# 666DZY666/micronet

Measured on AMD Instinct MI355X. Metric: QAT images/sec (nin_gc CIFAR-10, W-ternary/A-binary), higher is better.
Workload: dtype f32

## Files before the change

### include/micronet_hip.h

```cpp
#ifndef MICRONET_HIP_H
#define MICRONET_HIP_H

#include <stddef.h>
#include <stdint.h>

#ifdef __cplusplus
extern "C" {
#endif

#define MN_OK 0
#define MN_EINVAL (-22)
#define MN_ENOTSUP (-95)
#define MN_EHIP (-5)
#define MN_ENOSPC (-28)

typedef void* mn_stream_t;

int mn_version(void);
const char* mn_last_error(void);
const char* mn_last_kernel(void);
void mn_profile_next(void* start_event, void* stop_event);
typedef struct mn_prof_entry {
    char name[96];
    int64_t launches;
// ... 268 lines not shown
                                const float* sums, int training, const float* w, float* dx, void* ws, int64_t ws_bytes, mn_stream_t stream);
int mn_conv2d_bwd_weight_bnh_pool(const mn_conv_geom* g, const float* dpool, const uint8_t* h, const int8_t* own, const float* chan, const float* sums,
                                  int training, const int8_t* x, float* dw, float* dbias, void* ws, int64_t ws_bytes, mn_stream_t stream);
int mn_conv2d_bwd_bnh_supported(const mn_conv_geom* g, const mn_wq* wq, int pooled);
int64_t mn_conv2d_bwd_bnh_ws_bytes(const mn_conv_geom* g);
int mn_conv2d_bwd_bnh(const mn_conv_geom* g, const mn_wq* wq, const float* da, const uint8_t* h, const int8_t* own, const float* chan, const float* sums,
                      int training, const float* w, const int8_t* x, float* dx, float* dw, float* dbias, void* ws, int64_t ws_bytes, mn_stream_t stream);
int mn_conv2d_bwd_bnh_up_splits(const mn_conv_geom* g, const mn_wq* wq, int pooled, int64_t up_k);
int mn_conv2d_bwd_bnh_up(const mn_conv_geom* g, const mn_wq* wq, const float* da, const uint8_t* h, const int8_t* own, const float* chan, const float* sums,
                         int training, const float* w, const int8_t* x, float* dx, float* dw, float* dbias, void* ws, int64_t ws_bytes,
                         const uint8_t* up_h, const float* up_chan, double* up_part, mn_stream_t stream);
int mn_conv2d_bwd_bnh_up9_splits(const mn_conv_geom* g, const mn_wq* wq, int64_t up_k);
int mn_conv2d_bwd_bnh_up9(const mn_conv_geom* g, const mn_wq* wq, const float* da, const uint8_t* h, const float* chan, const float* sums, int training,
                          const float* w, const int8_t* x, float* dx, float* dw, float* dbias, void* ws, int64_t ws_bytes, const uint8_t* up_h, const float* up_chan,
                          double* up_part, mn_stream_t stream);
int mn_conv2d_bwd_codes(const mn_conv_geom* g, const mn_wq* wq, const float* gy, const float* w, const void* x_codes, int x_bits, float* dx, float* dw, float* dbias,
                        void* ws, int64_t ws_bytes, mn_stream_t stream);
int mn_conv2d_bwd_qa(const mn_conv_geom* g, const mn_wq* wq, const float* dq, const void* stash, int stash_bits, const float* chan, const float* sums, int out_bits,
                     int quant, int training, const float* w, const uint8_t* x_codes, int x_bits, float* dx, float* dw, float* dbias, void* ws, int64_t ws_bytes,
                     mn_stream_t stream);
int mn_conv2d_bwd_codes_up(const mn_conv_geom* g, const mn_wq* wq, const float* gy, const float* w, const void* x_codes, int x_bits, float* dx, float* dw, float* dbias,
                           void* ws, int64_t ws_bytes, const void* up_stash, const float* up_chan, int up_quant, double* up_part, mn_stream_t stream);
int mn_conv2d_bwd_qa_up(const mn_conv_geom* g, const mn_wq* wq, const float* dq, const void* stash, const float* chan, const float* sums, int out_bits, int quant,
                        int training, const float* w, const uint8_t* x_codes, int x_bits, float* dx, float* dw, float* dbias, void* ws, int64_t ws_bytes,
                        const void* up_stash, const float* up_chan, int up_quant, double* up_part, mn_stream_t stream);
int mn_qconv_bnsign_bwd_pooled(const mn_conv_geom* g, const mn_wq* wq, const int8_t* x, const float* w, const float* bias, const float* gamma,
                               const float* beta, const float* save, const float* dpool, const int8_t* a_own, int training, float* dy,
                               float* dgamma, float* dbeta, void* ws, int64_t ws_bytes, mn_stream_t stream);

#define MN_QA_NCH 9
// ... 118 lines not shown
```

### micronet_amd/_lib.py

```python
import ctypes as C
import os

HERE = os.path.dirname(os.path.abspath(__file__))
LIB_PATH = os.environ.get("MN_LIB_PATH") or os.path.join(HERE, "lib", "libmicronet_hip.so")

MN_ACTQ_NONE, MN_ACTQ_DOREFA, MN_ACTQ_IAO, MN_ACTQ_SIGN8, MN_ACTQ_CODE8 = 0, 1, 2, 3, 4
MN_ALGO_AUTO, MN_ALGO_DIRECT, MN_ALGO_MFMA, MN_ALGO_QGEMM = 0, 1, 2, 3
MN_WQ_REAL, MN_WQ_TERNARY, MN_WQ_DOREFA, MN_WQ_IAO = 0, 1, 2, 3
MN_ACTQ_X_IS_CODE = 1
MN_ACTQ_CODES_GIVEN = 2
MN_ENOTSUP = -95


class ConvGeom(C.Structure):
    _fields_ = [(n, C.c_int32) for n in ("N", "C", "H", "W", "O", "KH", "KW", "stride_h", "stride_w", "pad_h", "pad_w",
                                         "dil_h", "dil_w", "groups", "in_shuffle")]


class ActQ(C.Structure):
    _fields_ = [("mode", C.c_int32), ("bits", C.c_int32), ("q_type", C.c_int32), ("flags", C.c_int32),
                ("qp", C.c_void_p), ("codes", C.c_void_p), ("stats", C.c_void_p), ("dx_add", C.c_void_p), ("ste_mask", C.c_void_p), ("acc_mm", C.c_void_p)]


class WQ(C.Structure):
# ... 84 lines not shown
    "mn_qconv_bnsign_fwd_stash_pool_supported": (_I, [_G, _W]),
    "mn_qconv_bnsign_fwd_stash_pool": (_I, [_G, _W, _P, _P, _P, _P, _P, C.c_float, C.c_float, _I, _P, _P, _P, _P, _P, _P, _P, _P, _P, _L, _P]),
    "mn_bnh_bwd_sums": (_I, [_P, _P, _P, _P, _L, _L, _L, _L, _P, _P, _P, _P, _P]),
    "mn_bnh_bwd_apply": (_I, [_P, _P, _P, _P, _P, _L, _L, _L, _L, _I, _P, _P]),
    "mn_conv2d_bnh_supported": (_I, [_G, _W]),
    "mn_conv2d_bwd_data_bnh": (_I, [_G, _W, _P, _P, _P, _P, _I, _P, _P, _P, _L, _P]),
    "mn_conv2d_bwd_weight_bnh": (_I, [_G, _P, _P, _P, _P, _I, _P, _P, _P, _P, _L, _P]),
    "mn_conv2d_bwd_bnh_supported": (_I, [_G, _W, _I]),
    "mn_conv2d_bwd_bnh_ws_bytes": (_L, [_G]),
    "mn_conv2d_bwd_bnh": (_I, [_G, _W, _P, _P, _P, _P, _P, _I, _P, _P, _P, _P, _P, _P, _L, _P]),
    "mn_conv2d_bwd_bnh_up_splits": (_I, [_G, _W, _I, _L]),
    "mn_conv2d_bwd_bnh_up": (_I, [_G, _W, _P, _P, _P, _P, _P, _I, _P, _P, _P, _P, _P, _P, _L, _P, _P, _P, _P]),
    "mn_bnh_bwd_sums_final": (_I, [_P, _I, _L, _L, _L, _L, _P, _P, _P, _P]),
    "mn_conv2d_bwd_bnh_up9_splits": (_I, [_G, _W, _L]),
    "mn_conv2d_bwd_bnh_up9": (_I, [_G, _W, _P, _P, _P, _P, _I, _P, _P, _P, _P, _P, _P, _L, _P, _P, _P, _P]),
    "mn_conv2d_bwd_codes": (_I, [_G, _W, _P, _P, _P, _I, _P, _P, _P, _P, _L, _P]),
    "mn_conv2d_bwd_qa": (_I, [_G, _W, _P, _P, _I, _P, _P, _I, _I, _I, _P, _P, _I, _P, _P, _P, _P, _L, _P]),
    "mn_conv2d_bwd_codes_up": (_I, [_G, _W, _P, _P, _P, _I, _P, _P, _P, _P, _L, _P, _P, _I, _P, _P]),
    "mn_conv2d_bwd_qa_up": (_I, [_G, _W, _P, _P, _P, _P, _I, _I, _I, _P, _P, _I, _P, _P, _P, _P, _L, _P, _P, _I, _P, _P]),
    "mn_qa_bwd_sums_final": (_I, [_P, _I, _L, _P, _P, _P, _P]),
    "mn_conv2d_bnh_pool_supported": (_I, [_G, _W]),
    "mn_conv2d_bwd_data_bnh_pool": (_I, [_G, _W, _P, _P, _P, _P, _P, _I, _P, _P, _P, _L, _P]),
    "mn_conv2d_bwd_weight_bnh_pool": (_I, [_G, _P, _P, _P, _P, _P, _I, _P, _P, _P, _P, _L, _P]),
    "mn_qconv_bnsign_bwd": (_I, [_G, _W, _P, _P, _P, _P, _P, _P, _P, _I, _P, _P, _P, _P, _L, _P]),
    "mn_qconv_bnsign_bwd_pooled": (_I, [_G, _W, _P, _P, _P, _P, _P, _P, _P, _P, _I, _P, _P, _P, _P, _L, _P]),
    "mn_signconv1x1_small_supported": (_I, [_L, _L, _L]),
    "mn_signconv1x1_small_fwd": (_I, [_P, _P, _P, _P, _L, _L, _L, _L, _P]),
    "mn_codeconv1x1_small_fwd": (_I, [_P, _I, _P, _P, _P, _L, _L, _L, _L, _P]),
    "mn_conv1x1_small_bwd_data": (_I, [_P, _P, _P, _L, _L, _L, _L, _P]),
    "mn_iao_fq_act_fwd": (_I, [_P, _P, _L, _P, _I, _I, _I, C.c_float, _P]),
# ... 152 lines not shown
```

### micronet_amd/csrc/conv_kernels.hip

```cpp
#include "common.h"
#include "qgemm.h"

#define EPI_PLAIN 0
#define EPI_BIAS 1
#define EPI_STE 2

struct TileGeom {
    int TP, NI, TR, tpi;
    int PR, PW, HALO, CS;
    int num_ptiles;
    FastDiv fd_wo, fd_tr, fd_pwq, fd_pr, fd_ni, fd_tpi, fd_ppi;
    int tpq_shift;
};
struct ConvView {
    const float* in;
    int N, Cin_total, Hin, Win, U, Hv, Wv, Kc, G;
    int Cout_total, Ho, Wo, Mg;
    int KH, KW, Sh, Sw, Dh, Dw, ph, pw;
    int vec_in;
};
static inline int roundup(int a, int b) { return (a + b - 1) / b * b; }

static int make_tile_geom(const ConvView& v, int TP, int cs_mod32, TileGeom* t) {
    if (v.Wo < 4 || TP % v.Wo != 0 || v.pw > 8 || v.pw < 0 || v.ph < 0) return 0;
// ... 797 lines not shown
    return pwb_bwd_bnh_up(g, wq, da, h, own, chan, sums, training, w, x, dx, dw, dbias, ws, ws_bytes, up_h, up_chan, up_part, (hipStream_t)stream);
}
extern "C" int mn_conv2d_bwd_bnh_up9_splits(const mn_conv_geom* g, const mn_wq* wq, int64_t up_k) {
    if (check_geom(g, "mn_conv2d_bwd_bnh_up9_splits") != MN_OK) return 0;
    if (up_k < 1 || up_k > 254 || !pwb_supported(g, wq, 0)) return 0;
    return pwb_up9_splits(g);
}
extern "C" int mn_conv2d_bwd_bnh_up9(const mn_conv_geom* g, const mn_wq* wq, const float* da, const uint8_t* h, const float* chan, const float* sums, int training,
                                     const float* w, const int8_t* x, float* dx, float* dw, float* dbias, void* ws, int64_t ws_bytes, const uint8_t* up_h,
                                     const float* up_chan, double* up_part, mn_stream_t stream) {
    int rc = check_geom(g, "mn_conv2d_bwd_bnh_up9");
    if (rc) return rc;
    if (!wq || !da || !h || !chan || !sums || !w || !x || !dx || !dw || !up_h || !up_chan || !up_part) MN_FAIL(MN_EINVAL, "mn_conv2d_bwd_bnh_up9: null tensor");
    return pwb_bwd_bnh_up9(g, wq, da, h, chan, sums, training, w, x, dx, dw, dbias, ws, ws_bytes, up_h, up_chan, up_part, (hipStream_t)stream);
}
extern "C" int mn_conv2d_bwd_codes(const mn_conv_geom* g, const mn_wq* wq, const float* gy, const float* w, const void* x_codes, int x_bits, float* dx, float* dw,
                                   float* dbias, void* ws, int64_t ws_bytes, mn_stream_t stream) {
    int rc = check_geom(g, "mn_conv2d_bwd_codes");
    if (rc) return rc;
    if (!wq || !gy || !w || !x_codes || !dx || !dw || x_bits < 0 || x_bits > 8) MN_FAIL(MN_EINVAL, "mn_conv2d_bwd_codes: null tensor / bad bit width");
    return pwb_bwd_plain(g, wq, gy, w, x_codes, x_bits, dx, dw, dbias, ws, ws_bytes, (hipStream_t)stream);
}
extern "C" int mn_conv2d_bwd_qa(const mn_conv_geom* g, const mn_wq* wq, const float* dq, const void* stash, int stash_bits, const float* chan, const float* sums,
                                int out_bits, int quant, int training, const float* w, const uint8_t* x_codes, int x_bits, float* dx, float* dw, float* dbias, void* ws,
                                int64_t ws_bytes, mn_stream_t stream) {
    int rc = check_geom(g, "mn_conv2d_bwd_qa");
    if (rc) return rc;
    if (!wq || !dq || !stash || !chan || !sums || !w || !x_codes || !dx || !dw) MN_FAIL(MN_EINVAL, "mn_conv2d_bwd_qa: null tensor");
    return pwb_bwd_qa(g, wq, dq, stash, stash_bits, chan, sums, out_bits, quant, training, w, x_codes, x_bits, dx, dw, dbias, ws, ws_bytes, (hipStream_t)stream);
}
// ... 126 lines not shown
```

### micronet_amd/csrc/qgemm.h

```cpp
#pragma once
#include "common.h"

int qg_supported(const mn_conv_geom* g, const mn_actq* aq, const mn_wq* wq, int which);
int64_t qg_ws_bytes(const mn_conv_geom* g, int which);
int qg_fwd(const mn_conv_geom* g, const mn_actq* aq, const mn_wq* wq, const float* x, const float* w, const float* bias, float* y,
           void* ws, int64_t ws_bytes, hipStream_t s);
int qg_bwd_data(const mn_conv_geom* g, const mn_actq* aq, const mn_wq* wq, const float* gy, const float* w, const float* x, float* dx,
                void* ws, int64_t ws_bytes, hipStream_t s);
int qg_fwd_act_mm_count(const mn_conv_geom* g);
int qg_fwd_act(const mn_conv_geom* g, const mn_actq* aq, const mn_wq* wq, const float* x, const float* w, const float* bias, float* y, int relu, float* mm,
               void* ws, int64_t ws_bytes, hipStream_t s);
int c1_supported(const mn_conv_geom* g, int which);
int64_t c1_ws_bytes(const mn_conv_geom* g, int which);
int c1_fwd(const mn_conv_geom* g, const float* x, const float* w, const float* bias, float* y, void* ws, int64_t ws_bytes, hipStream_t s);
int c1_fwd_mm_count(const mn_conv_geom* g);
int c1_fwd_act(const mn_conv_geom* g, const float* x, const float* w, const float* bias, float* y, int relu, float* mm, void* ws, int64_t ws_bytes, hipStream_t s);
int c1_bwd_weight_bn(const mn_conv_geom* g, const float* gy, const float* da, const float* yb, const float* save, const float* gamma, const float* beta,
                     const float* sums, int training, const float* x, float* dw, float* dbias, void* ws, int64_t ws_bytes, hipStream_t s);
int c1_bwd_weight(const mn_conv_geom* g, const float* gy, const float* x, float* dw, float* dbias, void* ws, int64_t ws_bytes, hipStream_t s);
int c1_bwd_weight_qa(const mn_conv_geom* g, const float* dq, const float* yb, const float* chan, int quant, int a_bits, const float* sums, int training,
                     const float* x, float* dw, float* dbias, void* ws, int64_t ws_bytes, hipStream_t s);
int qd_iao_dx_add_supported(const mn_conv_geom* g, const mn_actq* aq, const mn_wq* wq);
int64_t qd_iao_ws_bytes(const mn_conv_geom* g, int which);
int qd_iao_bwd_data(const mn_conv_geom* g, const mn_actq* aq, const mn_wq* wq, const float* gy, const float* w, const float* x, float* dx, void* ws, int64_t ws_bytes,
// ... 29 lines not shown
int pwb_up_splits(const mn_conv_geom* g);
int pwb_bwd_bnh_up(const mn_conv_geom* g, const mn_wq* wq, const float* da, const uint8_t* h, const int8_t* own, const float* chan, const float* sums, int training,
                   const float* w, const int8_t* x, float* dx, float* dw, float* dbias, void* ws, int64_t ws_bytes, const uint8_t* up_h, const float* up_chan,
                   double* up_part, hipStream_t s);
int pwb_up9_splits(const mn_conv_geom* g);
int pwb_bwd_bnh_up9(const mn_conv_geom* g, const mn_wq* wq, const float* da, const uint8_t* h, const float* chan, const float* sums, int training, const float* w,
                    const int8_t* x, float* dx, float* dw, float* dbias, void* ws, int64_t ws_bytes, const uint8_t* up_h, const float* up_chan, double* up_part,
                    hipStream_t s);
int pwb_bwd_plain_up(const mn_conv_geom* g, const mn_wq* wq, const float* gy, const float* w, const void* x, int x_bits, float* dx, float* dw, float* dbias, void* ws,
                     int64_t ws_bytes, const void* up_stash, const float* up_chan, int up_quant, double* up_part, hipStream_t s);
int pwb_bwd_qa_up(const mn_conv_geom* g, const mn_wq* wq, const float* dq, const void* stash, const float* chan, const float* sums, int out_bits, int quant, int training,
                  const float* w, const uint8_t* x, int x_bits, float* dx, float* dw, float* dbias, void* ws, int64_t ws_bytes, const void* up_stash, const float* up_chan,
                  int up_quant, double* up_part, hipStream_t s);
int pwb_bwd_bnh(const mn_conv_geom* g, const mn_wq* wq, const float* da, const uint8_t* h, const int8_t* own, const float* chan, const float* sums, int training,
                const float* w, const int8_t* x, float* dx, float* dw, float* dbias, void* ws, int64_t ws_bytes, hipStream_t s);
int pwb_bwd_plain(const mn_conv_geom* g, const mn_wq* wq, const float* gy, const float* w, const void* x, int x_bits, float* dx, float* dw, float* dbias, void* ws,
                  int64_t ws_bytes, hipStream_t s);
int pwb_bwd_qa(const mn_conv_geom* g, const mn_wq* wq, const float* dq, const void* stash, int stash_bits, const float* chan, const float* sums, int out_bits, int quant,
               int training, const float* w, const uint8_t* x, int x_bits, float* dx, float* dw, float* dbias, void* ws, int64_t ws_bytes, hipStream_t s);
```

### micronet_amd/csrc/qgemm_k3s.hip

```cpp
#include "qgemm_dev.h"

#include <stdlib.h>

#define K3_RSA 160
#define K3_NXL 6

struct K3wParams {
    const float* gy;
    const char* x;
    float* part;
    float* dbpart;
    int N, C, H, W, O, Cg, Mg, G, nmb, ncb, Z, Mgw, Cgw, want_db;
    int R, spi, nsteps, st_per_z, DPC, W4, CS, XB;
    FastDiv fd_spi, fd_dpc, fd_w4;
    ChanMap in_map;
};

template <int XENC>
__global__ __launch_bounds__(256, 2) void k_k3s_wgrad(const K3wParams p) {
    HIP_DYNAMIC_SHARED(float, smem)
    const int tid = threadIdx.x, lane = tid & 63, wave = tid >> 6, j = lane & 15, kg = lane >> 4;
    unsigned char* gsm = reinterpret_cast<unsigned char*>(smem) + wave * (32 * K3_RSA + p.XB);
    unsigned char* xsm = gsm + 32 * K3_RSA;
    uint32_t b = blockIdx.x;
// ... 768 lines not shown
    p.wn = (float)((1ll << wq->bits) - 1);
    mn_set_last_kernel(wide ? "k_k3s_fwd<2>" : "k_k3s_fwd<1>");
    { const double nx = (double)g->N * g->C * g->H * g->W, ny = (double)g->N * g->O * g->H * g->W; mn_prof_bytes(nx + (wide ? 4.0 : 2.0) * ny); }
    mn_prof_begin(s);
    if (wide) {
        raise_lds_limit((const void*)k_k3s_fwd<2>, pl.lds);
        hipLaunchKernelGGL(k_k3s_fwd<2>, dim3(pl.grid), dim3(256), pl.lds, s, p);
    } else {
        raise_lds_limit((const void*)k_k3s_fwd<1>, pl.lds);
        hipLaunchKernelGGL(k_k3s_fwd<1>, dim3(pl.grid), dim3(256), pl.lds, s, p);
    }
    mn_prof_end(s);
    MN_CHECK_LAUNCH("mn_qconv_bnq_fwd_stash(3x3)");
    return MN_OK;
}
```

### micronet_amd/ops.py

```python
import ctypes as C
import threading
import weakref

import torch
from torch.autograd import Function

from . import _lib
from ._lib import ActQ, ConvGeom, MicronetHipError, WQ
from .sign_tensor import LazyBNAct, LazyBNGrad, LazyConvOut, LazyPoolGrad, LazyQConvOut, LazyReluConvOut, LazyReluGrad, QActTensor, QGrad, SignTensor

ACTQ_NONE, ACTQ_DOREFA, ACTQ_IAO, ACTQ_SIGN8, ACTQ_CODE8 = _lib.MN_ACTQ_NONE, _lib.MN_ACTQ_DOREFA, _lib.MN_ACTQ_IAO, _lib.MN_ACTQ_SIGN8, _lib.MN_ACTQ_CODE8
WQ_REAL, WQ_TERNARY, WQ_DOREFA, WQ_IAO = _lib.MN_WQ_REAL, _lib.MN_WQ_TERNARY, _lib.MN_WQ_DOREFA, _lib.MN_WQ_IAO

PROFILER = None


class _Span:
    __slots__ = ("tok",)

    def __init__(self, tok):
        self.tok = tok

    def __enter__(self):
        return self
# ... 1765 lines not shown


def _out_hw(g):
    return ((g.H + 2 * g.pad_h - g.dil_h * (g.KH - 1) - 1) // g.stride_h + 1,
            (g.W + 2 * g.pad_w - g.dil_w * (g.KW - 1) - 1) // g.stride_w + 1)


def _ws(g, which, device):
    nb = int(_lib_().mn_conv2d_ws_bytes(C.byref(g), which, _lib.MN_ALGO_AUTO))
    if nb < 0:
        raise MicronetHipError("invalid convolution geometry")
    return torch.empty(max(nb // 4, 4), dtype=torch.float32, device=device), nb


FUSE_PW_BWD = _os0.environ.get("MN_PWB", "1") != "0"


def _wq_desc(wdesc):
    if wdesc is None:
        return None
    mode, bits, q_type, per_channel, scale = wdesc
    return WQ(mode, bits, q_type, per_channel, scale.data_ptr() if scale is not None else None)


def _ref(d):
    return None if d is None else C.byref(d)


class UpSums:
    __slots__ = ("h", "chan", "k", "ready", "kind")
# ... 78 lines not shown
            elif _lib_().mn_conv2d_bwd_data_add_supported(C.byref(g), C.byref(aq), C.byref(wd)):
                ctx.res_tok = x._mn_res_token = ResidualToken()
        ctx.save_for_backward(x, wq, qp, wscale)
        ctx.cfg = (g, aq_mode, aq_bits, aq_qtype, bias is not None, wdesc[:4] if wdesc is not None else None, aq_flags)
        return y

    @staticmethod
    def backward(ctx, gy):
        x, wq, qp, wscale = ctx.saved_tensors
        g, aq_mode, aq_bits, aq_qtype, has_bias, wd4, aq_flags = ctx.cfg
        if isinstance(gy, LazyBNGrad) and gy._mn_value is None and gy._mn_recipe.get("kind") == "first_done":
            r = gy._mn_recipe
            if aq_mode == ACTQ_NONE and not ctx.needs_input_grad[0] and r["x"].data_ptr() == x.data_ptr() and r["w"].data_ptr() == wq.data_ptr() and \
                    tuple(r["dw"].shape) == tuple(wq.shape) and (not has_bias or r["db"] is not None):
                return None, r["dw"], (r["db"] if has_bias else None), None, None, None, None, None, None, None, None, None, None, None, None
        if isinstance(gy, LazyBNGrad) and gy._mn_value is None and gy._mn_recipe.get("kind") in ("bnh", "bnh_pool") and aq_mode == ACTQ_SIGN8 and wd4 is not None:
            r = gy._mn_recipe
            pool = r.get("kind") == "bnh_pool"
            wd = _wq_desc(wd4 + (wscale,))
            if getattr(ctx, "packed", None) is not None and ctx.packed[1] is not None:
                wd.packed_bwd = ctx.packed[1].data_ptr()
            dx = dw = db = None
            want_w = ctx.needs_input_grad[1] or (has_bias and ctx.needs_input_grad[2])
            if ctx.needs_input_grad[0] and want_w and FUSE_PW_BWD and _lib_().mn_conv2d_bwd_bnh_supported(C.byref(g), _ref(wd), 1 if pool else 0) and \
                    r["da"].data_ptr() % 16 == 0 and x.data_ptr() % 16 == 0:
                with torch.cuda.device_of(x):
                    dx = torch.empty(x.shape, dtype=torch.float32, device=x.device)
                    dw = torch.empty_like(wq)
                    db = torch.empty(g.O, dtype=torch.float32, device=x.device) if has_bias else None
                    nb = int(_lib_().mn_conv2d_bwd_bnh_ws_bytes(C.byref(g)))
                    ws = torch.empty(max(nb // 4, 4), dtype=torch.float32, device=x.device)
# ... 166 lines not shown
            wd.packed_fwd = pk[0].data_ptr()
        with torch.cuda.device_of(codes):
            nb = int(_lib_().mn_qconv_bnsign_stash_ws_bytes(C.byref(g)))
            ws = torch.empty(nb // 4 + 4, dtype=torch.float32, device=codes.device)
            ap = None
            if pool_next and training and POOL_IN_SIGN_PASS and a.data_ptr() % 16 == 0 and h.data_ptr() % 16 == 0 and \
                    _lib_().mn_qconv_bnsign_fwd_stash_pool_supported(C.byref(g), _ref(wd)):
                ap = torch.empty((y.shape[0], y.shape[1], y.shape[2] // 2, y.shape[3] // 2), dtype=torch.int8, device=codes.device)
                _call("mn_qconv_bnsign_fwd_stash_pool", C.byref(g), _ref(wd), _p(codes), _p(wq), _p(bias), _p(gamma), _p(beta), float(eps), float(momentum),
                      int(training), _p(running_mean), _p(running_var), _p(nbt), _p(save), _p(a), _p(ap), _p(h), _p(chan), _p(ws), nb, _s())
            else:
                _call("mn_qconv_bnsign_fwd_stash", C.byref(g), _ref(wd), _p(codes), _p(wq), _p(bias), _p(gamma), _p(beta), float(eps), float(momentum),
                      int(training), _p(running_mean), _p(running_var), _p(nbt), _p(save), _p(a), _p(h), _p(chan), _p(ws), nb, _s())
        ctx.save_for_backward(h, chan, gamma, beta)
        ctx.training = int(training)
        ctx.fold_ok = FOLD_BN_INTO_CONV_BWD and bool(_lib_().mn_conv2d_bnh_supported(C.byref(g), _ref(wd)))
        ctx.fold_pool_ok = ctx.fold_ok and bool(_lib_().mn_conv2d_bnh_pool_supported(C.byref(g), _ref(wd)))
        out = SignTensor(a)
        if ap is not None:
            out._mn_pooled = ap
        ctx.up_rec = None
        if chan.shape[0] in (8, 17) and UP_SUMS_FOLD:
            ctx.up_rec = out._mn_up = UpSums(h, chan, wq.shape[1] * wq.shape[2] * wq.shape[3], kind=1 if chan.shape[0] == 8 else 3)
        return out

    @staticmethod
    def backward(ctx, da):
        h, chan, gamma, beta = ctx.saved_tensors
        training = ctx.training
        pooled = isinstance(da, LazyPoolGrad) and da._mn_value is None
        if pooled:
            grad, own = da._mn_pg, da._mn_codes
# ... 15 lines not shown
                _call("mn_bnh_bwd_sums", _p(grad), _p(h), _p(own), _p(chan), N, Cc, H, W, _p(dgamma), _p(dbeta), _p(sums), _p(ws), _s())
            if pooled and getattr(ctx, "fold_pool_ok", False) and LAZY_BN_GRAD:
                def expand_p(r):
                    dy_ = torch.empty(r["h"].shape, dtype=torch.float32, device=r["h"].device)
                    with torch.cuda.device_of(dy_):
                        _call("mn_bnh_bwd_apply", _p(r["da"]), _p(r["h"]), _p(r["own"]), _p(r["chan"]), _p(r["sums"]), N, Cc, H, W, r["training"], _p(dy_), _s())
                    return dy_
                recipe = dict(kind="bnh_pool", da=grad, own=own, h=h, chan=chan, sums=sums, training=training)
                return LazyBNGrad(h.shape, h.device, recipe, expand_p), dgamma, dbeta, None, None, None, None, None, None, None
            if not pooled and ctx.fold_ok and LAZY_BN_GRAD:
                def expand(r):
                    dy_ = torch.empty(r["h"].shape, dtype=torch.float32, device=r["h"].device)
                    with torch.cuda.device_of(dy_):
                        _call("mn_bnh_bwd_apply", _p(r["da"]), _p(r["h"]), None, _p(r["chan"]), _p(r["sums"]), N, Cc, H, W, r["training"], _p(dy_), _s())
                    return dy_
                recipe = dict(kind="bnh", da=grad, h=h, chan=chan, sums=sums, training=training)
                return LazyBNGrad(h.shape, h.device, recipe, expand), dgamma, dbeta, None, None, None, None, None, None, None
            dy = torch.empty(h.shape, dtype=torch.float32, device=h.device)
            _call("mn_bnh_bwd_apply", _p(grad), _p(h), _p(own), _p(chan), _p(sums), N, Cc, H, W, training, _p(dy), _s())
        return dy, dgamma, dbeta, None, None, None, None, None, None, None


def qconv_bnq_supported(x, wq, stride, padding, dilation, groups, w_bits, in_shuffle):
    if not isinstance(x, QActTensor) or x.dim() != 4 or not (2 <= w_bits <= 8):
        return False
    one = lambda v: v in (1, (1, 1), [1, 1])
    if not one(dilation):
        return False
    g = _geom(x.shape, wq.shape, stride, padding, dilation, groups, in_shuffle or 0)
    wd = WQ(WQ_DOREFA, w_bits, 0, 0, None)
    return bool(_lib_().mn_qconv_bnq_supported(C.byref(g), C.byref(wd), x.bits))
# ... 835 lines not shown
```

Before: 145,000.

## Fuse BN-backward apply into 3x3 ternary conv backward data and weight kernel

Adds a fused kernel for 3x3 stride-1 grouped ternary convolutions. It rebuilds the BN/hardtanh input gradient from the stashed codes and per-channel stats inside the conv backward, then computes dx through bf16 MFMA with a three-way bf16 split, while other waves accumulate weight-gradient partials. The Python side marks eligible BN layers so the lazy BN gradient is never materialized for them. This removes a full-size float dy write and read plus separate dgrad/wgrad launches, at the cost of a large specialized kernel with narrow geometry limits and a high LDS footprint.

```diff
diff --git a/include/micronet_hip.h b/include/micronet_hip.h
--- a/include/micronet_hip.h
+++ b/include/micronet_hip.h
@@ -306,6 +306,10 @@
 int mn_conv2d_bwd_bnh_up9(const mn_conv_geom* g, const mn_wq* wq, const float* da, const uint8_t* h, const float* chan, const float* sums, int training,
                           const float* w, const int8_t* x, float* dx, float* dw, float* dbias, void* ws, int64_t ws_bytes, const uint8_t* up_h, const float* up_chan,
                           double* up_part, mn_stream_t stream);
+int mn_conv2d_bwd_bnh_k3_supported(const mn_conv_geom* g, const mn_wq* wq);
+int64_t mn_conv2d_bwd_bnh_k3_ws_bytes(const mn_conv_geom* g);
+int mn_conv2d_bwd_bnh_k3(const mn_conv_geom* g, const mn_wq* wq, const float* da, const uint8_t* h, const float* chan, const float* sums, int training,
+                         const float* w, const int8_t* x, float* dx, float* dw, float* dbias, void* ws, int64_t ws_bytes, mn_stream_t stream);
 int mn_conv2d_bwd_codes(const mn_conv_geom* g, const mn_wq* wq, const float* gy, const float* w, const void* x_codes, int x_bits, float* dx, float* dw, float* dbias,
                         void* ws, int64_t ws_bytes, mn_stream_t stream);
 int mn_conv2d_bwd_qa(const mn_conv_geom* g, const mn_wq* wq, const float* dq, const void* stash, int stash_bits, const float* chan, const float* sums, int out_bits,
diff --git a/micronet_amd/_lib.py b/micronet_amd/_lib.py
--- a/micronet_amd/_lib.py
+++ b/micronet_amd/_lib.py
@@ -122,6 +122,9 @@
     "mn_bnh_bwd_sums_final": (_I, [_P, _I, _L, _L, _L, _L, _P, _P, _P, _P]),
     "mn_conv2d_bwd_bnh_up9_splits": (_I, [_G, _W, _L]),
     "mn_conv2d_bwd_bnh_up9": (_I, [_G, _W, _P, _P, _P, _P, _I, _P, _P, _P, _P, _P, _P, _L, _P, _P, _P, _P]),
+    "mn_conv2d_bwd_bnh_k3_supported": (_I, [_G, _W]),
+    "mn_conv2d_bwd_bnh_k3_ws_bytes": (_L, [_G]),
+    "mn_conv2d_bwd_bnh_k3": (_I, [_G, _W, _P, _P, _P, _P, _I, _P, _P, _P, _P, _P, _P, _L, _P]),
     "mn_conv2d_bwd_codes": (_I, [_G, _W, _P, _P, _P, _I, _P, _P, _P, _P, _L, _P]),
     "mn_conv2d_bwd_qa": (_I, [_G, _W, _P, _P, _I, _P, _P, _I, _I, _I, _P, _P, _I, _P, _P, _P, _P, _L, _P]),
     "mn_conv2d_bwd_codes_up": (_I, [_G, _W, _P, _P, _P, _I, _P, _P, _P, _P, _L, _P, _P, _I, _P, _P]),
diff --git a/micronet_amd/csrc/conv_kernels.hip b/micronet_amd/csrc/conv_kernels.hip
--- a/micronet_amd/csrc/conv_kernels.hip
+++ b/micronet_amd/csrc/conv_kernels.hip
@@ -835,6 +835,21 @@
     if (!wq || !da || !h || !chan || !sums || !w || !x || !dx || !dw || !up_h || !up_chan || !up_part) MN_FAIL(MN_EINVAL, "mn_conv2d_bwd_bnh_up9: null tensor");
     return pwb_bwd_bnh_up9(g, wq, da, h, chan, sums, training, w, x, dx, dw, dbias, ws, ws_bytes, up_h, up_chan, up_part, (hipStream_t)stream);
 }
+extern "C" int mn_conv2d_bwd_bnh_k3_supported(const mn_conv_geom* g, const mn_wq* wq) {
+    if (check_geom(g, "mn_conv2d_bwd_bnh_k3_supported") != MN_OK) return 0;
+    return k3b_supported(g, wq);
+}
+extern "C" int64_t mn_conv2d_bwd_bnh_k3_ws_bytes(const mn_conv_geom* g) {
+    if (check_geom(g, "mn_conv2d_bwd_bnh_k3_ws_bytes") != MN_OK) return -1;
+    return k3b_ws_bytes(g);
+}
+extern "C" int mn_conv2d_bwd_bnh_k3(const mn_conv_geom* g, const mn_wq* wq, const float* da, const uint8_t* h, const float* chan, const float* sums, int training,
+                                    const float* w, const int8_t* x, float* dx, float* dw, float* dbias, void* ws, int64_t ws_bytes, mn_stream_t stream) {
+    int rc = check_geom(g, "mn_conv2d_bwd_bnh_k3");
+    if (rc) return rc;
+    if (!wq || !da || !h || !chan || !sums || !w || !x || !dx || !dw) MN_FAIL(MN_EINVAL, "mn_conv2d_bwd_bnh_k3: null tensor");
+    return k3b_bwd_bnh(g, wq, da, h, chan, sums, training, w, x, dx, dw, dbias, ws, ws_bytes, (hipStream_t)stream);
+}
 extern "C" int mn_conv2d_bwd_codes(const mn_conv_geom* g, const mn_wq* wq, const float* gy, const float* w, const void* x_codes, int x_bits, float* dx, float* dw,
                                    float* dbias, void* ws, int64_t ws_bytes, mn_stream_t stream) {
     int rc = check_geom(g, "mn_conv2d_bwd_codes");
diff --git a/micronet_amd/csrc/qgemm.h b/micronet_amd/csrc/qgemm.h
--- a/micronet_amd/csrc/qgemm.h
+++ b/micronet_amd/csrc/qgemm.h
@@ -67,6 +67,10 @@
                   int up_quant, double* up_part, hipStream_t s);
 int pwb_bwd_bnh(const mn_conv_geom* g, const mn_wq* wq, const float* da, const uint8_t* h, const int8_t* own, const float* chan, const float* sums, int training,
                 const float* w, const int8_t* x, float* dx, float* dw, float* dbias, void* ws, int64_t ws_bytes, hipStream_t s);
+int k3b_supported(const mn_conv_geom* g, const mn_wq* wq);
+int64_t k3b_ws_bytes(const mn_conv_geom* g);
+int k3b_bwd_bnh(const mn_conv_geom* g, const mn_wq* wq, const float* da, const uint8_t* h, const float* chan, const float* sums, int training, const float* w,
+                const int8_t* x, float* dx, float* dw, float* dbias, void* ws, int64_t ws_bytes, hipStream_t s);
 int pwb_bwd_plain(const mn_conv_geom* g, const mn_wq* wq, const float* gy, const float* w, const void* x, int x_bits, float* dx, float* dw, float* dbias, void* ws,
                   int64_t ws_bytes, hipStream_t s);
 int pwb_bwd_qa(const mn_conv_geom* g, const mn_wq* wq, const float* dq, const void* stash, int stash_bits, const float* chan, const float* sums, int out_bits, int quant,
diff --git a/micronet_amd/csrc/qgemm_k3s.hip b/micronet_amd/csrc/qgemm_k3s.hip
--- a/micronet_amd/csrc/qgemm_k3s.hip
+++ b/micronet_amd/csrc/qgemm_k3s.hip
@@ -806,3 +806,423 @@
     MN_CHECK_LAUNCH("mn_qconv_bnq_fwd_stash(3x3)");
     return MN_OK;
 }
+
+#define K3B_FR 20
+
+struct K3bParams {
+    const float* da;
+    const unsigned char* h;
+    const float* chan;
+    const float* sums;
+    const char* x;
+    const float* w;
+    float* dx;
+    float* part;
+    float* dbpart;
+    int N, C, H, W, O, Cg, Mg, G, Z, training, want_db;
+    float n_f;
+    int NI, SP, HW, IS, TS, WP, RS32;
+    int nsteps, st_per_z, spi;
+    FastDiv fd_hw4, fd_w4, fd_w;
+    ChanMap in_map;
+};
+
+__global__ __launch_bounds__(512, 1) void k_k3b(const K3bParams p) {
+    HIP_DYNAMIC_SHARED(float, smem)
+    unsigned char* lds = reinterpret_cast<unsigned char*>(smem);
+    unsigned char* dyr = lds + 3 * p.TS;
+    float* ftab = reinterpret_cast<float*>(dyr + 32 * p.RS32);
+    const int tid = threadIdx.x, lane = tid & 63, wave = mn_uniform(tid >> 6), j = lane & 15, kg = lane >> 4;
+    const int role = wave >> 2, rw = wave & 3;
+    const uint32_t b = blockIdx.x;
+    const int z = (int)(b % (uint32_t)p.Z);
+    const int g = (int)(b / (uint32_t)p.Z);
+    const int wrow = p.Cg * 9;
+
+    float* wl = reinterpret_cast<float*>(lds);
+    for (int i = tid; i < p.Mg * wrow; i += 512) wl[i] = p.w[(int64_t)g * p.Mg * wrow + i];
+    __syncthreads();
+    float my_alpha = 0.f;
+    u32x4 wa[9];
+    if (role == 0) {
+        {
+            const int m = tid >> 3, part = tid & 7;
+            float a = 0.f;
+            if (m < p.Mg) for (int k = part; k < wrow; k += 8) a = fmaxf(a, fabsf(wl[m * wrow + k]));
+            a = fmaxf(a, __shfl_xor(a, 4, 64)); a = fmaxf(a, __shfl_xor(a, 2, 64)); a = fmaxf(a, __shfl_xor(a, 1, 64));
+            my_alpha = a;
+        }
+        const int c = j;
+#pragma unroll
+        for (int t = 0; t < 9; ++t) {
+            uint32_t h16[8];
+#pragma unroll
+            for (int e = 0; e < 8; ++e) {
+                const int m = 2 * kg + (e >> 2) + 8 * (e & 3);
+                float v = 0.f;
+                if (m < p.Mg && c < p.Cg) v = wl[m * wrow + c * 9 + t];
+                h16[e] = v > 0.f ? 0x3F80u : (v < 0.f ? 0xBF80u : 0u);
+            }
+            wa[t] = u32x4{h16[0] | (h16[1] << 16), h16[2] | (h16[3] << 16), h16[4] | (h16[5] << 16), h16[6] | (h16[7] << 16)};
+        }
+    }
+    __syncthreads();
+    for (int i = tid; i < (3 * p.TS) / 16; i += 512) *reinterpret_cast<u32x4*>(lds + 16 * i) = u32x4{0u, 0u, 0u, 0u};
+    if (role == 0 && (tid & 7) == 0) {
+        const int m = tid >> 3, co = g * p.Mg + (m < p.Mg ? m : p.Mg - 1), O = p.O;
+        float* fr = ftab + m * K3B_FR;
+        const StashNnz zn = stash_nnz_load(p.chan, O, co);
+        const bool ok = m < p.Mg;
+        fr[0] = ok ? p.chan[O + co] : 0.f; fr[1] = ok ? p.chan[2 * O + co] : 1.f; fr[2] = ok ? p.chan[3 * O + co] : 0.f;
+        fr[3] = ok ? p.chan[4 * O + co] : 0.f; fr[4] = ok ? p.chan[5 * O + co] : 0.f; fr[5] = ok ? p.chan[6 * O + co] : 0.f;
+        fr[6] = (ok && p.training) ? p.sums[co] / p.n_f : 0.f; fr[7] = (ok && p.training) ? p.sums[O + co] / p.n_f : 0.f;
+        fr[8] = zn.v0; fr[9] = zn.v1; fr[10] = zn.v2; fr[11] = zn.v3; fr[12] = zn.v4; fr[13] = zn.v5; fr[14] = zn.v6; fr[15] = zn.v7; fr[16] = zn.v8;
+        fr[17] = ok ? my_alpha : 0.f;
+    }
+    const int st0 = z * p.st_per_z;
+    const int st1 = (st0 + p.st_per_z < p.nsteps ? st0 + p.st_per_z : p.nsteps);
+    const int sg0 = st1 > st0 ? st0 / p.spi / p.NI : 0;
+    const int nst = st1 > st0 ? (st1 - 1) / p.spi / p.NI - sg0 + 1 : 0;
+    const int ntile = p.SP >> 5;
+    auto gstep = [&](int stg, int tile) -> int {
+        const int sp = tile * 32;
+        const int img = (int)fd_div((uint32_t)(sp >> 2), p.fd_hw4);
+        return (stg * p.NI + img) * p.spi + ((sp - img * p.HW) >> 5);
+    };
+
+    const int cps = p.SP >> 2;
+    const bool sact = tid < 8 * cps;
+    int s_slot, s_img, s_nz[3], s_row;
+    uint32_t s_goff[4];
+    {
+        const int chunk = tid % cps, sr = (tid / cps) & 7;
+        const uint32_t img = fd_div(chunk, p.fd_hw4);
+        const int q = chunk - (int)img * (p.HW >> 2);
+        const uint32_t row = fd_div(q, p.fd_w4);
+        const int col = (q - (int)row * (p.W >> 2)) * 4;
+        s_slot = ((int)img * p.IS + ((int)row + 1) * p.WP + col + 1) * K3D_RS + 8 * sr;
+        s_row = sr * p.RS32 + 16 * chunk;
+        s_img = (int)img;
+        const int rc = row == 0 ? 0 : ((int)row == p.H - 1 ? 2 : 1);
+        s_nz[0] = 8 + 3 * rc + (col == 0 ? 0 : 1);
+        s_nz[1] = 8 + 3 * rc + 1;
+        s_nz[2] = 8 + 3 * rc + (col + 3 == p.W - 1 ? 2 : 1);
+#pragma unroll
+        for (int i = 0; i < 4; ++i) {
+            int m = sr + 8 * i;
+            m = m < p.Mg ? m : p.Mg - 1;
+            s_goff[i] = (img * (uint32_t)p.O + (uint32_t)(g * p.Mg + m)) * (uint32_t)p.HW + 4u * q;
+        }
+    }
+    const bool cact = tid < cps * 4;
+    int c_slot, c_img;
+    uint32_t c_goff[4];
+    bool c_cv[4];
+    {
+        const int chunk = tid % cps, csr = (tid / cps) & 3;
+        const uint32_t img = fd_div(chunk, p.fd_hw4);
+        const int q = chunk - (int)img * (p.HW >> 2);
+        const uint32_t row = fd_div(q, p.fd_w4);
+        const int col = (q - (int)row * (p.W >> 2)) * 4;
+        c_slot = (csr >> 1) * p.TS + ((int)img * p.IS + ((int)row + 1) * p.WP + col + 1) * K3D_RS + 64 + 8 * (csr & 1);
+        c_img = (int)img;
+#pragma unroll
+        for (int i = 0; i < 4; ++i) {
+            const int c = csr + 4 * i;
+            c_cv[i] = c < p.Cg;
+            c_goff[i] = (img * (uint32_t)p.C + (uint32_t)chan_phys(p.in_map, g * p.Cg + (c_cv[i] ? c : p.Cg - 1))) * (uint32_t)p.HW + 4u * q;
+        }
+    }
+    float4 rg[4];
+    uint32_t hg[4], xg[4];
+    auto fetch = [&](int st) {
+        const int64_t lim = ((int64_t)p.N * p.O - 1) * p.HW + p.HW - 4;
+#pragma unroll
+        for (int i = 0; i < 4; ++i) {
+            int64_t off = (int64_t)st * p.NI * p.O * p.HW + s_goff[i];
+            off = off < lim ? off : lim;
+            rg[i] = *reinterpret_cast<const float4*>(p.da + off);
+            hg[i] = *reinterpret_cast<const uint32_t*>(p.h + off);
+        }
+        const int64_t limx = ((int64_t)p.N * p.C - 1) * p.HW + p.HW - 4;
+#pragma unroll
+        for (int i = 0; i < 4; ++i) {
+            int64_t off = (int64_t)st * p.NI * p.C * p.HW + c_goff[i];
+            off = off < limx ? off : limx;
+            xg[i] = *reinterpret_cast<const uint32_t*>(p.x + off);
+        }
+    };
+    auto commit = [&](int st) {
+        if (sact) {
+            const int sr = (tid / cps) & 7;
+            const bool valid = st * p.NI + s_img < p.N;
+#pragma unroll
+            for (int ip = 0; ip < 2; ++ip) {
+                float t0[2][4], t1[2][4], t2[2][4];
+#pragma unroll
+                for (int ii = 0; ii < 2; ++ii) {
+                    const int i = 2 * ip + ii;
+                    const float* fr = ftab + (sr + 8 * i) * K3B_FR;
+                    const float fl = fr[0], L = fr[1], U = fr[2], A = fr[3], B = fr[4], gi = fr[5], k1 = fr[6], k2 = fr[7], al = fr[17];
+                    const float nz[4] = {fr[s_nz[0]], fr[s_nz[1]], fr[s_nz[1]], fr[s_nz[2]]};
+                    const float gv[4] = {rg[i].x, rg[i].y, rg[i].z, rg[i].w};
+                    float dv[4], v[4];
+#pragma unroll
+                    for (int e = 0; e < 4; ++e) {
+                        const float acc = 2.f * (float)((hg[i] >> (8 * e)) & 0xffu) - nz[e];
+                        const float uu = acc * fl;
+                        const float dz = (uu >= L && uu <= U) ? gv[e] : 0.f;
+                        const float dy = gi * (dz - k1 - fmaf(acc, A, B) * k2);
+                        dv[e] = valid ? dy : 0.f;
+                        v[e] = dv[e] * al;
+                    }
+                    *reinterpret_cast<float4*>(dyr + s_row + 8 * i * p.RS32) = make_float4(dv[0], dv[1], dv[2], dv[3]);
+#pragma unroll
+                    for (int e = 0; e < 4; ++e) {
+                        t0[ii][e] = mn_bf16_head(v[e]);
+                        const float r1 = v[e] - t0[ii][e];
+                        t1[ii][e] = mn_bf16_head(r1);
+                        t2[ii][e] = r1 - t1[ii][e];
+                    }
+                }
+#pragma unroll
+                for (int e = 0; e < 4; ++e) {
+                    unsigned char* d = lds + s_slot + e * K3D_RS + 4 * ip;
+                    *reinterpret_cast<uint32_t*>(d) = mn_pack_bf16x2(t0[0][e], t0[1][e]);
+                    *reinterpret_cast<uint32_t*>(d + p.TS) = mn_pack_bf16x2(t1[0][e], t1[1][e]);
+                    *reinterpret_cast<uint32_t*>(d + 2 * p.TS) = mn_pack_bf16x2(t2[0][e], t2[1][e]);
+                }
+            }
+        }
+        if (cact) {
+            const bool valid = st * p.NI + c_img < p.N;
+            uint32_t en[4];
+#pragma unroll
+            for (int i = 0; i < 4; ++i) en[i] = (c_cv[i] && valid) ? ((xg[i] & 0x80808080u) | 0x3F3F3F3Fu) : 0u;
+#pragma unroll
+            for (int e = 0; e < 4; ++e) {
+                const uint32_t se = 0x000c000cu | ((uint32_t)e << 8) | ((uint32_t)(4 + e) << 24);
+                *reinterpret_cast<u32x2*>(lds + c_slot + e * K3D_RS) = u32x2{mn_perm(en[1], en[0], se), mn_perm(en[3], en[2], se)};
+            }
+        }
+    };
+    if (nst > 0) fetch(sg0);
+    f32x4 accw[2][9];
+    float dbacc[4] = {0.f, 0.f, 0.f, 0.f};
+    if (role == 0) {
+        for (int k = 0; k < nst; ++k) {
+            const int st = sg0 + k;
+            __syncthreads();
+            commit(st);
+            __syncthreads();
+            fetch(k + 1 < nst ? st + 1 : st);
+            for (int tile = rw; tile < ntile; tile += 4) {
+                const int gs = gstep(st, tile);
+                if (gs < st0 || gs >= st1) continue;
+                f32x4 acc[2][3];
+#pragma unroll
+                for (int hh = 0; hh < 2; ++hh)
+#pragma unroll
+                    for (int t = 0; t < 3; ++t) acc[hh][t] = f32x4{0.f, 0.f, 0.f, 0.f};
+                int sb[2], opp[2], oimg[2];
+#pragma unroll
+                for (int hh = 0; hh < 2; ++hh) {
+                    const int sp = tile * 32 + hh * 16 + j;
+                    const uint32_t img = fd_div(sp >> 2, p.fd_hw4);
+                    const int pp = sp - (int)img * p.HW;
+                    const uint32_t row = fd_div(pp, p.fd_w);
+                    const int col = pp - (int)row * p.W;
+                    sb[hh] = ((int)img * p.IS + ((int)row + 1) * p.WP + col + 1) * K3D_RS + 16 * kg;
+                    opp[hh] = pp; oimg[hh] = (int)img;
+                }
+#pragma unroll
+                for (int r = 0; r < 3; ++r)
+#pragma unroll
+                    for (int s_ = 0; s_ < 3; ++s_) {
+                        const int toff = ((1 - r) * p.WP + (1 - s_)) * K3D_RS;
+#pragma unroll
+                        for (int t = 0; t < 3; ++t)
+#pragma unroll
+                            for (int hh = 0; hh < 2; ++hh) {
+                                const u32x4 bf = *reinterpret_cast<const u32x4*>(lds + t * p.TS + sb[hh] + toff);
+                                acc[hh][t] = mn_mfma_bf16(wa[r * 3 + s_], bf, acc[hh][t]);
+                            }
+                    }
+#pragma unroll
+                for (int hh = 0; hh < 2; ++hh) {
+                    const int n = st * p.NI + oimg[hh];
+#pragma unroll
+                    for (int rr = 0; rr < 4; ++rr) {
+                        const int c = 4 * kg + rr;
+                        if (n < p.N && c < p.Cg)
+                            p.dx[((int64_t)n * p.C + chan_phys(p.in_map, g * p.Cg + c)) * p.HW + opp[hh]] = (acc[hh][0][rr] + acc[hh][1][rr]) + acc[hh][2][rr];
+                    }
+                }
+            }
+        }
+    } else {
+#pragma unroll
+        for (int mi = 0; mi < 2; ++mi)
+#pragma unroll
+            for (int t = 0; t < 9; ++t) accw[mi][t] = f32x4{0.f, 0.f, 0.f, 0.f};
+        const int e4 = j >> 2, q4 = j & 3;
+        const int cpos = (q4 >> 1) * p.TS + 64 + 8 * (q4 & 1);
+        const int sr = lane >> 3, sq = lane & 7;
+        for (int k = 0; k < nst; ++k) {
+            const int st = sg0 + k;
+            __syncthreads();
+            commit(st);
+            __syncthreads();
+            fetch(k + 1 < nst ? st + 1 : st);
+            for (int tile = 0; tile < ntile; ++tile) {
+                const int gs = gstep(st, tile);
+                if (gs < st0 || gs >= st1 || ((gs - st0) & 3) != rw) continue;
+#pragma unroll
+                for (int i = 0; i < 4; ++i) {
+                    const float4 gv = *reinterpret_cast<const float4*>(dyr + (sr + 8 * i) * p.RS32 + 4 * (tile * 32 + 4 * sq));
+                    dbacc[i] += (gv.x + gv.y) + (gv.z + gv.w);
+                }
+                u32x4 a0[2], a1[2], a2[2];
+#pragma unroll
+                for (int mi = 0; mi < 2; ++mi) {
+                    const unsigned char* row = dyr + (mi * 16 + j) * p.RS32 + 4 * (tile * 32 + 4 * kg);
+                    const float4 ga = *reinterpret_cast<const float4*>(row), gb = *reinterpret_cast<const float4*>(row + 64);
+                    const float v[8] = {ga.x, ga.y, ga.z, ga.w, gb.x, gb.y, gb.z, gb.w};
+                    float t0[8], t1[8], t2[8];
+#pragma unroll
+                    for (int e = 0; e < 8; ++e) {
+                        t0[e] = mn_bf16_head(v[e]);
+                        const float r1 = v[e] - t0[e];
+                        t1[e] = mn_bf16_head(r1);
+                        t2[e] = r1 - t1[e];
+                    }
+#pragma unroll
+                    for (int d = 0; d < 4; ++d) {
+                        a0[mi][d] = mn_pack_bf16x2(t0[2 * d], t0[2 * d + 1]);
+                        a1[mi][d] = mn_pack_bf16x2(t1[2 * d], t1[2 * d + 1]);
+                        a2[mi][d] = mn_pack_bf16x2(t2[2 * d], t2[2 * d + 1]);
+                    }
+                }
+                int sl[2];
+#pragma unroll
+                for (int hb = 0; hb < 2; ++hb) {
+                    const int sp = tile * 32 + 16 * hb + 4 * kg + e4;
+                    const uint32_t img = fd_div(sp >> 2, p.fd_hw4);
+                    const int pp = sp - (int)img * p.HW;
+                    const uint32_t row = fd_div(pp, p.fd_w);
+                    sl[hb] = ((int)img * p.IS + ((int)row + 1) * p.WP + (pp - (int)row * p.W) + 1) * K3D_RS + cpos;
+                }
+#pragma unroll
+                for (int r = 0; r < 3; ++r) {
+                    u32x4 bf[3];
+#pragma unroll
+                    for (int s_ = 0; s_ < 3; ++s_) {
+                        const int toff = ((r - 1) * p.WP + (s_ - 1)) * K3D_RS;
+                        const mn_u32x2 lo = mn_lds_tr16_b64(lds + sl[0] + toff);
+                        const mn_u32x2 hi = mn_lds_tr16_b64(lds + sl[1] + toff);
+                        bf[s_] = u32x4{lo[0], lo[1], hi[0], hi[1]};
+                    }
+#pragma unroll
+                    for (int s_ = 0; s_ < 3; ++s_)
+#pragma unroll
+                        for (int mi = 0; mi < 2; ++mi) accw[mi][r * 3 + s_] = mn_mfma_bf16(a0[mi], bf[s_], accw[mi][r * 3 + s_]);
+#pragma unroll
+                    for (int s_ = 0; s_ < 3; ++s_)
+#pragma unroll
+                        for (int mi = 0; mi < 2; ++mi) accw[mi][r * 3 + s_] = mn_mfma_bf16(a1[mi], bf[s_], accw[mi][r * 3 + s_]);
+#pragma unroll
+                    for (int s_ = 0; s_ < 3; ++s_)
+#pragma unroll
+                        for (int mi = 0; mi < 2; ++mi) accw[mi][r * 3 + s_] = mn_mfma_bf16(a2[mi], bf[s_], accw[mi][r * 3 + s_]);
+                }
+            }
+        }
+    }
+    float* red = smem;
+    float* dbs = smem + 32 * 144;
+    for (int w_ = 0; w_ < 4; ++w_) {
+        __syncthreads();
+        if (role == 1 && rw == w_) {
+#pragma unroll
+            for (int mi = 0; mi < 2; ++mi)
+#pragma unroll
+                for (int t = 0; t < 9; ++t)
+#pragma unroll
+                    for (int r = 0; r < 4; ++r) {
+                        const int idx = (mi * 16 + kg * 4 + r) * 144 + ((j >> 2) + 4 * (j & 3)) * 9 + t;
+                        red[idx] = (w_ == 0) ? accw[mi][t][r] : red[idx] + accw[mi][t][r];
+                    }
+#pragma unroll
+            for (int i = 0; i < 4; ++i) {
+                float v = dbacc[i];
+                v += __shfl_xor(v, 4, 64); v += __shfl_xor(v, 2, 64); v += __shfl_xor(v, 1, 64);
+                if ((lane & 7) == 0) dbs[(lane >> 3) + 8 * i] = (w_ == 0) ? v : dbs[(lane >> 3) + 8 * i] + v;
+            }
+        }
+    }
+    __syncthreads();
+    float* dst = p.part + ((int64_t)z * p.G + g) * (32 * 144);
+    for (int i = tid; i < 32 * 144; i += 512) dst[i] = red[i];
+    if (p.want_db && tid < 32) p.dbpart[((int64_t)z * p.G + g) * 32 + tid] = dbs[tid];
+}
+
+struct K3bPlan { K3bParams p; int grid; size_t lds; int64_t off_db, ws_bytes; };
+static int plan_k3b(const mn_conv_geom* g, const mn_wq* wq, K3bPlan* pl) {
+    if (wq && wq->mode != MN_WQ_TERNARY) return 0;
+    if (g->KH != 3 || g->KW != 3 || g->stride_h != 1 || g->stride_w != 1 || g->pad_h != 1 || g->pad_w != 1 || g->dil_h != 1 || g->dil_w != 1) return 0;
+    if (g->in_shuffle > 1 && g->C % g->in_shuffle) return 0;
+    if (g->groups < 1 || g->C % g->groups || g->O % g->groups) return 0;
+    const int HW = g->H * g->W, Mg = g->O / g->groups, Cg = g->C / g->groups;
+    if (g->W % 4 || HW % 32 || g->H < 2 || Mg > 32 || Mg < 1 || Cg > 16 || Cg < 1) return 0;
+    if ((int64_t)g->N * g->O * HW >= ((int64_t)1 << 31) || (int64_t)g->N * g->C * HW >= ((int64_t)1 << 31)) return 0;
+    K3wPlan wp;
+    if (!plan_k3s(g, &wp) || wp.p.nmb != 1 || wp.p.ncb != 1 || wp.p.R * g->W != 32) return 0;
+    K3bParams& p = pl->p;
+    int NI = 1;
+    while (NI * HW < 128) NI *= 2;
+    const int SP = NI * HW;
+    if (SP > 256 || SP % 128) return 0;
+    p.N = g->N; p.C = g->C; p.H = g->H; p.W = g->W; p.O = g->O; p.Cg = Cg; p.Mg = Mg; p.G = g->groups;
+    p.NI = NI; p.SP = SP; p.HW = HW; p.WP = g->W + 2; p.IS = (g->H + 2) * (g->W + 2);
+    p.TS = (NI * p.IS * K3D_RS + 255) / 256 * 256;
+    p.RS32 = SP * 4 + 16;
+    p.Z = wp.p.Z; p.nsteps = wp.p.nsteps; p.st_per_z = wp.p.st_per_z; p.spi = wp.p.spi;
+    if (p.spi * 32 != HW) return 0;
+    const size_t lds = (size_t)3 * p.TS + (size_t)32 * p.RS32 + 32 * K3B_FR * 4;
+    const size_t wimg = (size_t)Mg * Cg * 9 * 4, epi = (size_t)(32 * 144 + 32) * 4;
+    if ((size_t)3 * p.TS < wimg || (size_t)3 * p.TS < epi) return 0;
+    if (lds > 160 * 1024) return 0;
+    pl->lds = lds;
+    const int64_t nb = (int64_t)p.G * p.Z;
+    if (nb > 0x7fffffff) return 0;
+    pl->grid = (int)nb;
+    p.fd_hw4 = make_fastdiv((uint32_t)(HW / 4)); p.fd_w4 = make_fastdiv((uint32_t)(g->W / 4)); p.fd_w = make_fastdiv((uint32_t)g->W);
+    p.in_map = make_chanmap(g->in_shuffle, g->C);
+    p.n_f = (float)g->N * (float)HW;
+    const int64_t part_bytes = (int64_t)p.Z * p.G * 32 * 144 * 4;
+    pl->off_db = (part_bytes + 255) / 256 * 256;
+    pl->ws_bytes = pl->off_db + (int64_t)p.Z * p.G * 32 * 4;
+    return 1;
+}
+int k3b_supported(const mn_conv_geom* g, const mn_wq* wq) { K3bPlan pl; return wq && plan_k3b(g, wq, &pl); }
+int64_t k3b_ws_bytes(const mn_conv_geom* g) { K3bPlan pl; return plan_k3b(g, nullptr, &pl) ? pl.ws_bytes : 0; }
+int k3b_bwd_bnh(const mn_conv_geom* g, const mn_wq* wq, const float* da, const uint8_t* h, const float* chan, const float* sums, int training, const float* w,
+                const int8_t* x, float* dx, float* dw, float* dbias, void* ws, int64_t ws_bytes, hipStream_t s) {
+    K3bPlan pl;
+    if (!wq || !plan_k3b(g, wq, &pl)) MN_FAIL(MN_ENOTSUP, "mn_conv2d_bwd_bnh_k3: geometry / quantizer combination not covered");
+    if (!aligned16(da) || (((uintptr_t)h) & 3) || (((uintptr_t)x) & 3) || (((uintptr_t)dx) & 3) || (((uintptr_t)dw) & 3)) MN_FAIL(MN_ENOTSUP, "mn_conv2d_bwd_bnh_k3: misaligned tensor");
+    if (!ws || ws_bytes < pl.ws_bytes || !aligned16(ws)) MN_FAIL(MN_ENOSPC, "mn_conv2d_bwd_bnh_k3: workspace too small");
+    K3bParams& p = pl.p;
+    p.da = da; p.h = h; p.chan = chan; p.sums = sums; p.x = (const char*)x; p.w = w; p.dx = dx;
+    p.part = (float*)ws; p.dbpart = (float*)((char*)ws + pl.off_db);
+    p.training = training; p.want_db = dbias != nullptr;
+    mn_set_last_kernel("k_k3b");
+    { const double nx = (double)g->N * g->C * g->H * g->W, ny = (double)g->N * g->O * g->H * g->W; mn_prof_bytes(5.0 * ny + 5.0 * nx); }
+    mn_prof_begin(s);
+    raise_lds_limit((const void*)k_k3b, pl.lds);
+    hipLaunchKernelGGL(k_k3b, dim3(pl.grid), dim3(512), pl.lds, s, p);
+    mn_prof_end(s);
+    qg_launch_wgrad_reduce(p.part, p.dbpart, dw, dbias, p.Z, p.G, p.Mg, p.Cg * 9, 32, 144, 2.f, nullptr, s);
+    MN_CHECK_LAUNCH("mn_conv2d_bwd_bnh_k3");
+    return MN_OK;
+}
diff --git a/micronet_amd/ops.py b/micronet_amd/ops.py
--- a/micronet_amd/ops.py
+++ b/micronet_amd/ops.py
@@ -1803,6 +1803,7 @@
 
 
 FUSE_PW_BWD = _os0.environ.get("MN_PWB", "1") != "0"
+FUSE_K3_BWD = _os0.environ.get("MN_K3B", "1") != "0"
 
 
 def _wq_desc(wdesc):
@@ -1911,7 +1912,23 @@
             if aq_mode == ACTQ_NONE and not ctx.needs_input_grad[0] and r["x"].data_ptr() == x.data_ptr() and r["w"].data_ptr() == wq.data_ptr() and \
                     tuple(r["dw"].shape) == tuple(wq.shape) and (not has_bias or r["db"] is not None):
                 return None, r["dw"], (r["db"] if has_bias else None), None, None, None, None, None, None, None, None, None, None, None, None
-        if isinstance(gy, LazyBNGrad) and gy._mn_value is None and gy._mn_recipe.get("kind") in ("bnh", "bnh_pool") and aq_mode == ACTQ_SIGN8 and wd4 is not None:
+        if isinstance(gy, LazyBNGrad) and gy._mn_value is None and gy._mn_recipe.get("kind") == "bnh" and gy._mn_recipe.get("k3"):
+            r = gy._mn_recipe
+            want_w = ctx.needs_input_grad[1] or (has_bias and ctx.needs_input_grad[2])
+            wd = _wq_desc(wd4 + (wscale,)) if wd4 is not None else None
+            if aq_mode == ACTQ_SIGN8 and wd is not None and ctx.needs_input_grad[0] and want_w and \
+                    _lib_().mn_conv2d_bwd_bnh_k3_supported(C.byref(g), C.byref(wd)) and r["da"].data_ptr() % 16 == 0 and x.data_ptr() % 16 == 0:
+                with torch.cuda.device_of(x):
+                    dx = torch.empty(x.shape, dtype=torch.float32, device=x.device)
+                    dw = torch.empty_like(wq)
+                    db = torch.empty(g.O, dtype=torch.float32, device=x.device) if has_bias else None
+                    nb = int(_lib_().mn_conv2d_bwd_bnh_k3_ws_bytes(C.byref(g)))
+                    ws = torch.empty(max(nb // 4, 4), dtype=torch.float32, device=x.device)
+                    with _span(g, 1, 5 * r["h"].numel() + 5 * dx.numel()):
+                        _call("mn_conv2d_bwd_bnh_k3", C.byref(g), C.byref(wd), _p(r["da"]), _p(r["h"]), _p(r["chan"]), _p(r["sums"]), r["training"], _p(wq), _p(x),
+                              _p(dx), _p(dw), _p(db), _p(ws), nb, _s())
+                return dx, dw, db, None, None, None, None, None, None, None, None, None, None, None, None
+        elif isinstance(gy, LazyBNGrad) and gy._mn_value is None and gy._mn_recipe.get("kind") in ("bnh", "bnh_pool") and aq_mode == ACTQ_SIGN8 and wd4 is not None:
             r = gy._mn_recipe
             pool = r.get("kind") == "bnh_pool"
             wd = _wq_desc(wd4 + (wscale,))
@@ -2108,8 +2125,10 @@
                       int(training), _p(running_mean), _p(running_var), _p(nbt), _p(save), _p(a), _p(h), _p(chan), _p(ws), nb, _s())
         ctx.save_for_backward(h, chan, gamma, beta)
         ctx.training = int(training)
-        ctx.fold_ok = FOLD_BN_INTO_CONV_BWD and bool(_lib_().mn_conv2d_bnh_supported(C.byref(g), _ref(wd)))
-        ctx.fold_pool_ok = ctx.fold_ok and bool(_lib_().mn_conv2d_bnh_pool_supported(C.byref(g), _ref(wd)))
+        pw_fold = FOLD_BN_INTO_CONV_BWD and bool(_lib_().mn_conv2d_bnh_supported(C.byref(g), _ref(wd)))
+        ctx.fold_pool_ok = pw_fold and bool(_lib_().mn_conv2d_bnh_pool_supported(C.byref(g), _ref(wd)))
+        ctx.k3_fold = FOLD_BN_INTO_CONV_BWD and FUSE_K3_BWD and chan.shape[0] == 17 and bool(_lib_().mn_conv2d_bwd_bnh_k3_supported(C.byref(g), _ref(wd)))
+        ctx.fold_ok = pw_fold or ctx.k3_fold
         out = SignTensor(a)
         if ap is not None:
             out._mn_pooled = ap
@@ -2155,7 +2174,7 @@
                     with torch.cuda.device_of(dy_):
                         _call("mn_bnh_bwd_apply", _p(r["da"]), _p(r["h"]), None, _p(r["chan"]), _p(r["sums"]), N, Cc, H, W, r["training"], _p(dy_), _s())
                     return dy_
-                recipe = dict(kind="bnh", da=grad, h=h, chan=chan, sums=sums, training=training)
+                recipe = dict(kind="bnh", da=grad, h=h, chan=chan, sums=sums, training=training, k3=ctx.k3_fold)
                 return LazyBNGrad(h.shape, h.device, recipe, expand), dgamma, dbeta, None, None, None, None, None, None, None
             dy = torch.empty(h.shape, dtype=torch.float32, device=h.device)
             _call("mn_bnh_bwd_apply", _p(grad), _p(h), _p(own), _p(chan), _p(sums), N, Cc, H, W, training, _p(dy), _s())
```

Result: no change. 146,300 (median of 6 runs) (+0.9%).
